# mbzuai-oryx/Video-LLaVA

Measured on NVIDIA H100. Metric: videos/sec (100-frame CLIP encode + 7B 32-tok decode), higher is better.
Workload: dtype bf16

## Files before the change

### video-llava_b200/csrc/attention_tc.cu

```cuda
#include "common.cuh"
#include "kernels.h"

#include <stdlib.h>

namespace vcl {

namespace {

constexpr int VA_WG = 2;
constexpr int VA_THREADS = VA_WG * 128;
constexpr int VA_TILE = 64 * 128;
constexpr int VA_KEY_TILES = 5;
constexpr int VA_OFF_K = 0;
constexpr int VA_OFF_VT = VA_OFF_K + VA_KEY_TILES * VA_TILE;
constexpr int VA_OFF_Q = VA_OFF_VT + VA_KEY_TILES * VA_TILE;
constexpr int VA_OFF_P = VA_OFF_Q + VA_WG * VA_TILE;
constexpr int VA_OFF_BAR = VA_OFF_P + VA_WG * VA_KEY_TILES * VA_TILE;
constexpr int VA_SMEM = VA_OFF_BAR + 64 + 1024;
static_assert(VA_SMEM <= 227 * 1024, "shared memory");

__device__ __forceinline__ uint32_t va_sw128(int row, int chunk) {
  return (uint32_t)row * 128u + (uint32_t)((chunk ^ (row & 7)) << 4);
}

__device__ __forceinline__ void named_bar_sync_wg(int id) { asm volatile("bar.sync %0, 128;" ::"r"(id) : "memory"); }

__global__ void __launch_bounds__(VA_THREADS, 1)
attn_vit_tc_kernel(const __grid_constant__ CUtensorMap tmap, const bf16* __restrict__ qkv, bf16* __restrict__ out,
                   int S, int H, int C) {
  extern __shared__ uint8_t smem_raw[];
  const uint32_t raw_addr = smem_u32(smem_raw);
  const uint32_t pad = ((raw_addr + 1023u) & ~1023u) - raw_addr;
  uint8_t* smem = smem_raw + pad;
  const uint32_t sbase = raw_addr + pad;
  const uint32_t kbar = sbase + VA_OFF_BAR;
  auto qbar = [&](int w) { return sbase + VA_OFF_BAR + 8u * (1 + w); };

  const int frame = blockIdx.x / H, h = blockIdx.x - frame * H;
  const int row0 = frame * S;
  const int wg = threadIdx.x >> 7, t = threadIdx.x & 127, lane = threadIdx.x & 31, wq = t >> 5;
  const int n_qt = (S + 63) / 64;
  const int n_kt = (S + 63) / 64;

  if (threadIdx.x == 0) {
    tma_prefetch_desc(&tmap);
    mbar_init(kbar, 1);
    for (int w = 0; w < VA_WG; ++w) mbar_init(qbar(w), 1);
    mbar_fence_init();
  }
  __syncthreads();
  if (threadIdx.x == 0) {
    mbar_arrive_expect_tx(kbar, n_kt * VA_TILE);
    for (int i = 0; i < n_kt; ++i) tma_load_2d(sbase + VA_OFF_K + i * VA_TILE, &tmap, kbar, C + h * 64, row0 + 64 * i);
    for (int w = 0; w < VA_WG && w < n_qt; ++w) {
      mbar_arrive_expect_tx(qbar(w), VA_TILE);
      tma_load_2d(sbase + VA_OFF_Q + w * VA_TILE, &tmap, qbar(w), h * 64, row0 + 64 * w);
    }
  }
  const bf16* vg = qkv + (long long)row0 * 3 * C + 2 * C + h * 64;
  for (int idx = threadIdx.x; idx < VA_KEY_TILES * 64 * 8; idx += VA_THREADS) {
    const int key = idx % (VA_KEY_TILES * 64), c = idx / (VA_KEY_TILES * 64);
    uint4 v = make_uint4(0u, 0u, 0u, 0u);
    if (key < S) v = *reinterpret_cast<const uint4*>(vg + (long long)key * 3 * C + c * 8);
    const uint32_t w4[4] = {v.x, v.y, v.z, v.w};
    uint8_t* tile = smem + VA_OFF_VT + (key >> 6) * VA_TILE;
    const int kc = (key & 63) >> 3, ke = key & 7;
#pragma unroll
    for (int e = 0; e < 8; ++e) {
      const uint16_t hv = (uint16_t)(e & 1 ? w4[e >> 1] >> 16 : w4[e >> 1] & 0xffffu);
      *reinterpret_cast<uint16_t*>(tile + va_sw128(c * 8 + e, kc) + ke * 2) = hv;
    }
  }
  asm volatile("fence.proxy.async.shared::cta;" ::: "memory");
  __syncthreads();
  mbar_wait(kbar, 0);

  const int r0 = 16 * wq + (lane >> 2), c2 = 2 * (lane & 3);
  const bool tail = S > 256;
  uint8_t* P = smem + VA_OFF_P + wg * VA_KEY_TILES * VA_TILE;
  const uint32_t p_addr = sbase + VA_OFF_P + wg * VA_KEY_TILES * VA_TILE;
  const uint32_t q_addr = sbase + VA_OFF_Q + wg * VA_TILE;
  uint32_t qphase = 0;
  float s[128], s2[16], o[32];
  for (int qt = wg; qt < n_qt; qt += VA_WG) {
    mbar_wait(qbar(wg), qphase);
    qphase ^= 1u;
#pragma unroll
    for (int i = 0; i < 128; ++i) s[i] = 0.f;
#pragma unroll
    for (int i = 0; i < 16; ++i) s2[i] = 0.f;
    wgmma_fence();
#pragma unroll
    for (int k = 0; k < 4; ++k) {
      const uint64_t ad = wgmma_desc_k_sw128(q_addr) + 2u * k;
      wgmma_bf16<256>(s, ad, wgmma_desc_k_sw128(sbase + VA_OFF_K) + 2u * k, k > 0 ? 1u : 0u);
      if (tail) wgmma_bf16<32>(s2, ad, wgmma_desc_k_sw128(sbase + VA_OFF_K + 256 * 128) + 2u * k, k > 0 ? 1u : 0u);
    }
    wgmma_commit();
    wgmma_wait<0>();
    wgmma_fence_regs(s);
    wgmma_fence_regs(s2);
    named_bar_sync_wg(1 + wg);
    if (t == 0 && qt + VA_WG < n_qt) {
      mbar_arrive_expect_tx(qbar(wg), VA_TILE);
      tma_load_2d(q_addr, &tmap, qbar(wg), h * 64, row0 + 64 * (qt + VA_WG));
    }
    auto sc = [&](float x, int key) { return key < S ? bf16r(bf16r(x) * 0.125f) : -INFINITY; };
    float m[2] = {-INFINITY, -INFINITY};
    uint32_t sp[64], sp2[8];
    auto pack_sc = [&](const float* a, int i, int key0) {
      const int hh = i & 1, col = key0 + 8 * (i >> 1) + c2;
      const float x0 = sc(a[2 * i], col), x1 = sc(a[2 * i + 1], col + 1);
      m[hh] = fmaxf(m[hh], fmaxf(x0, x1));
      return pack_bf16x2(x0, x1);
    };
    if (tail) {
#pragma unroll
      for (int i = 0; i < 8; ++i) sp2[i] = pack_sc(s2, i, 256);
    }
#pragma unroll
    for (int i = 0; i < 64; ++i) sp[i] = pack_sc(s, i, 0);
    float l[2] = {0.f, 0.f};
#pragma unroll
    for (int r = 0; r < 2; ++r) {
      m[r] = fmaxf(m[r], __shfl_xor_sync(0xffffffffu, m[r], 1));
      m[r] = fmaxf(m[r], __shfl_xor_sync(0xffffffffu, m[r], 2));
    }
    auto put_p = [&](uint32_t x2, int i, int key0) {
      const int hh = i & 1, row = r0 + 8 * hh, col = key0 + 8 * (i >> 1) + c2;
      const float p0 = exp2f((bf16lo(x2) - m[hh]) * 1.4426950408889634f);
      const float p1 = exp2f((bf16hi(x2) - m[hh]) * 1.4426950408889634f);
      l[hh] += p0 + p1;
      *reinterpret_cast<uint32_t*>(P + (col >> 6) * VA_TILE + va_sw128(row, (col & 63) >> 3) + (col & 7) * 2) =
          pack_bf16x2(p0, p1);
    };
#pragma unroll
    for (int i = 0; i < 64; ++i) put_p(sp[i], i, 0);
    if (tail) {
#pragma unroll
      for (int i = 0; i < 8; ++i) put_p(sp2[i], i, 256);
    }
    asm volatile("fence.proxy.async.shared::cta;" ::: "memory");
    named_bar_sync_wg(1 + wg);
#pragma unroll
    for (int i = 0; i < 32; ++i) o[i] = 0.f;
    wgmma_fence();
#pragma unroll
    for (int kk = 0; kk < 16; ++kk)
      wgmma_bf16<64>(o, wgmma_desc_k_sw128(p_addr + (kk >> 2) * VA_TILE) + 2u * (kk & 3),
                     wgmma_desc_k_sw128(sbase + VA_OFF_VT + (kk >> 2) * VA_TILE) + 2u * (kk & 3), kk > 0 ? 1u : 0u);
    if (tail)
      wgmma_bf16<64>(o, wgmma_desc_k_sw128(p_addr + 4 * VA_TILE), wgmma_desc_k_sw128(sbase + VA_OFF_VT + 4 * VA_TILE), 1u);
    wgmma_commit();
    wgmma_wait<0>();
    wgmma_fence_regs(o);
#pragma unroll
    for (int r = 0; r < 2; ++r) {
      l[r] += __shfl_xor_sync(0xffffffffu, l[r], 1);
      l[r] += __shfl_xor_sync(0xffffffffu, l[r], 2);
    }
#pragma unroll
    for (int hh = 0; hh < 2; ++hh) {
      const int q = qt * 64 + r0 + 8 * hh;
      if (q < S) {
        const float inv = 1.0f / l[hh];
        bf16* dst = out + (long long)(row0 + q) * C + h * 64 + c2;
#pragma unroll
        for (int j = 0; j < 8; ++j)
          *reinterpret_cast<uint32_t*>(dst + 8 * j) = pack_bf16x2(o[4 * j + 2 * hh] * inv, o[4 * j + 2 * hh + 1] * inv);
      }
    }
  }
}

}

int init_attention_tc_kernels() {
  VCL_CUDA_OK(cudaFuncSetAttribute(attn_vit_tc_kernel, cudaFuncAttributeMaxDynamicSharedMemorySize, VA_SMEM));
  return 0;
}

bool attention_vit_tc_supported(int S) {
  const bool off = getenv("VCL_VIT_ATTN_FLASH") != nullptr;
  return !off && S >= 129 && S <= 257;
}

int launch_attention_vit_tc(const bf16* qkv, bf16* out, int n_frames, int S, int H, int C, cudaStream_t stream) {
  VCL_REQUIRE(C == H * 64, "attention_vit_tc: head_dim must be 64");
  VCL_REQUIRE(S >= 129 && S <= 257, "attention_vit_tc: S=%d outside 129..257", S);
  VCL_REQUIRE(((uintptr_t)qkv % 16) == 0 && ((uintptr_t)out % 16) == 0, "attention_vit_tc: pointers must be 16-byte aligned");
  CUtensorMap tm;
  if (make_tmap_2d(&tm, qkv, (long long)n_frames * S, 3LL * C, 3LL * C, 64) != 0) return -2;
  attn_vit_tc_kernel<<<n_frames * H, VA_THREADS, VA_SMEM, stream>>>(tm, qkv, out, S, H, C);
  VCL_CUDA_OK(cudaGetLastError());
  count_launches(1);
  return 0;
}

}
```

### video-llava_b200/csrc/common.cuh

```cuda
#pragma once

#include <cuda.h>
#include <cuda_bf16.h>
#include <cuda_fp16.h>
#include <cuda_runtime.h>
#include <stdint.h>

namespace vcl {

typedef __nv_bfloat16 bf16;

void set_last_error(const char* fmt, ...);

#define VCL_CUDA_OK(expr)                                                                      \
  do {                                                                                         \
    cudaError_t _e = (expr);                                                                   \
    if (_e != cudaSuccess) {                                                                   \
      ::vcl::set_last_error("%s:%d: %s -> %s", __FILE__, __LINE__, #expr, cudaGetErrorString(_e)); \
      return -2;                                                                               \
    }                                                                                          \
  } while (0)

#define VCL_REQUIRE(cond, ...)                 \
  do {                                         \
    if (!(cond)) {                             \
      ::vcl::set_last_error(__VA_ARGS__);      \
      return -1;                               \
    }                                          \
  } while (0)

__device__ __forceinline__ float bf16r(float x) { return __bfloat162float(__float2bfloat16_rn(x)); }

__device__ __forceinline__ uint32_t pack_bf16x2(float lo, float hi) {
  __nv_bfloat162 v = __floats2bfloat162_rn(lo, hi);
  return *reinterpret_cast<uint32_t*>(&v);
}
__device__ __forceinline__ float act_sigmoid_div(float num, float x) {
  const float d = 1.0f + __expf(-x);
  const float s = d > 0x1p126f ? 0.25f : 1.0f;
  return __fdividef(num * s, d * s);
}
__device__ __forceinline__ float bf16lo(uint32_t v) { return __uint_as_float(v << 16); }
__device__ __forceinline__ float bf16hi(uint32_t v) { return __uint_as_float(v & 0xffff0000u); }

__device__ __forceinline__ uint32_t bf16x2_mul(uint32_t a, uint32_t b) {
  __nv_bfloat162 r = __hmul2(*reinterpret_cast<__nv_bfloat162*>(&a), *reinterpret_cast<__nv_bfloat162*>(&b));
  return *reinterpret_cast<uint32_t*>(&r);
}
__device__ __forceinline__ uint32_t bf16x2_add(uint32_t a, uint32_t b) {
  __nv_bfloat162 r = __hadd2(*reinterpret_cast<__nv_bfloat162*>(&a), *reinterpret_cast<__nv_bfloat162*>(&b));
  return *reinterpret_cast<uint32_t*>(&r);
}

__device__ __forceinline__ float warp_sum(float v) {
#pragma unroll
  for (int o = 16; o > 0; o >>= 1) v += __shfl_xor_sync(0xffffffffu, v, o);
  return v;
}
__device__ __forceinline__ float warp_max(float v) {
#pragma unroll
  for (int o = 16; o > 0; o >>= 1) v = fmaxf(v, __shfl_xor_sync(0xffffffffu, v, o));
  return v;
}

__device__ __forceinline__ uint4 ld_nc_v4(const void* p) {
  uint4 r;
  asm volatile("ld.global.nc.L1::no_allocate.v4.u32 {%0,%1,%2,%3}, [%4];"
               : "=r"(r.x), "=r"(r.y), "=r"(r.z), "=r"(r.w)
               : "l"(p));
  return r;
}

__device__ __forceinline__ uint32_t smem_u32(const void* p) {
  return static_cast<uint32_t>(__cvta_generic_to_shared(p));
}

__device__ __forceinline__ void mbar_init(uint32_t bar, uint32_t count) {
  asm volatile("mbarrier.init.shared::cta.b64 [%0], %1;" ::"r"(bar), "r"(count) : "memory");
}
__device__ __forceinline__ void mbar_fence_init() {
  asm volatile("fence.mbarrier_init.release.cluster;" ::: "memory");
  asm volatile("fence.proxy.async.shared::cta;" ::: "memory");
}
__device__ __forceinline__ void mbar_arrive_expect_tx(uint32_t bar, uint32_t bytes) {
  asm volatile("mbarrier.arrive.expect_tx.shared::cta.b64 _, [%0], %1;" ::"r"(bar), "r"(bytes)
               : "memory");
}
__device__ __forceinline__ void mbar_arrive(uint32_t bar) {
  asm volatile("mbarrier.arrive.shared::cta.b64 _, [%0];" ::"r"(bar) : "memory");
}
__device__ __forceinline__ void mbar_wait(uint32_t bar, uint32_t parity) {
  asm volatile(
      "{\n\t"
      ".reg .pred p;\n\t"
      "VCL_WAIT_%=:\n\t"
      "mbarrier.try_wait.parity.shared::cta.b64 p, [%0], %1;\n\t"
      "@p bra VCL_DONE_%=;\n\t"
      "bra VCL_WAIT_%=;\n\t"
      "VCL_DONE_%=:\n\t"
      "}\n" ::"r"(bar),
      "r"(parity)
      : "memory");
}

__device__ __forceinline__ void tma_prefetch_desc(const void* tmap) {
  asm volatile("prefetch.tensormap [%0];" ::"l"(tmap) : "memory");
}
__device__ __forceinline__ void tma_load_2d(uint32_t dst_smem, const void* tmap, uint32_t bar,
                                            int32_t c0, int32_t c1) {
  asm volatile(
      "cp.async.bulk.tensor.2d.shared::cluster.global.mbarrier::complete_tx::bytes"
      " [%0], [%1, {%3, %4}], [%2];" ::"r"(dst_smem),
      "l"(tmap), "r"(bar), "r"(c0), "r"(c1)
      : "memory");
}

__device__ __forceinline__ void tma_prefetch_2d(const void* tmap, int32_t c0, int32_t c1) {
  asm volatile("cp.async.bulk.prefetch.tensor.2d.L2.global.tile [%0, {%1, %2}];" ::"l"(tmap), "r"(c0), "r"(c1)
               : "memory");
}

__device__ __forceinline__ void tma_load_2d_mc(uint32_t dst_smem, const void* tmap, uint32_t bar,
                                               int32_t c0, int32_t c1, uint16_t cta_mask) {
  asm volatile(
      "cp.async.bulk.tensor.2d.shared::cluster.global.mbarrier::complete_tx::bytes.multicast::cluster"
      " [%0], [%1, {%3, %4}], [%2], %5;" ::"r"(dst_smem),
      "l"(tmap), "r"(bar), "r"(c0), "r"(c1), "h"(cta_mask)
      : "memory");
}

__device__ __forceinline__ uint32_t cluster_ctarank() {
  uint32_t r;
  asm volatile("mov.u32 %0, %%cluster_ctarank;" : "=r"(r));
  return r;
}
__device__ __forceinline__ void cluster_sync_all() {
  asm volatile("barrier.cluster.arrive.release.aligned;" ::: "memory");
  asm volatile("barrier.cluster.wait.acquire.aligned;" ::: "memory");
}

__device__ __forceinline__ uint32_t mapa_cluster(uint32_t smem_addr, uint32_t cta_rank) {
  uint32_t r;
  asm volatile("mapa.shared::cluster.u32 %0, %1, %2;" : "=r"(r) : "r"(smem_addr), "r"(cta_rank));
  return r;
}
__device__ __forceinline__ void mbar_arrive_cluster(uint32_t bar_cluster_addr) {
  asm volatile("mbarrier.arrive.release.cluster.shared::cluster.b64 _, [%0];" ::"r"(bar_cluster_addr) : "memory");
}

__device__ __forceinline__ void wgmma_fence() { asm volatile("wgmma.fence.sync.aligned;" ::: "memory"); }
__device__ __forceinline__ void wgmma_commit() { asm volatile("wgmma.commit_group.sync.aligned;" ::: "memory"); }
template <int N>
__device__ __forceinline__ void wgmma_wait() {
  asm volatile("wgmma.wait_group.sync.aligned %0;" ::"n"(N) : "memory");
}
template <int R>
__device__ __forceinline__ void wgmma_fence_regs(float (&d)[R]) {
#pragma unroll
  for (int i = 0; i < R; ++i) asm volatile("" : "+f"(d[i])::"memory");
}
template <int R>
__device__ __forceinline__ void setmaxnreg_inc() { asm volatile("setmaxnreg.inc.sync.aligned.u32 %0;" ::"n"(R)); }
template <int R>
__device__ __forceinline__ void setmaxnreg_dec() { asm volatile("setmaxnreg.dec.sync.aligned.u32 %0;" ::"n"(R)); }

__device__ __forceinline__ uint64_t wgmma_desc_k_sw128(uint32_t smem_addr) {
  uint64_t d = 0;
  d |= (uint64_t)((smem_addr & 0x3ffffu) >> 4);
  d |= (uint64_t)1 << 16;
  d |= (uint64_t)(1024u >> 4) << 32;
  d |= (uint64_t)1 << 62;
  return d;
}

template <int N>
__device__ __forceinline__ void wgmma_bf16(float (&d)[N / 2], uint64_t adesc, uint64_t bdesc, uint32_t accumulate);
template <>
__device__ __forceinline__ void wgmma_bf16<256>(float (&d)[128], uint64_t adesc, uint64_t bdesc, uint32_t accumulate) {
  asm volatile(
      "{\n\t.reg .pred p;\n\tsetp.ne.b32 p, %130, 0;\n\t"
      "wgmma.mma_async.sync.aligned.m64n256k16.f32.bf16.bf16 {%0, %1, %2, %3, %4, %5, %6, %7, %8, %9, %10, %11, %12, %13, %14, %15, %16, %17, %18, %19, %20, %21, %22, %23, %24, %25, %26, %27, %28, %29, %30, %31, %32, %33, %34, %35, %36, %37, %38, %39, %40, %41, %42, %43, %44, %45, %46, %47, %48, %49, %50, %51, %52, %53, %54, %55, %56, %57, %58, %59, %60, %61, %62, %63, %64, %65, %66, %67, %68, %69, %70, %71, %72, %73, %74, %75, %76, %77, %78, %79, %80, %81, %82, %83, %84, %85, %86, %87, %88, %89, %90, %91, %92, %93, %94, %95, %96, %97, %98, %99, %100, %101, %102, %103, %104, %105, %106, %107, %108, %109, %110, %111, %112, %113, %114, %115, %116, %117, %118, %119, %120, %121, %122, %123, %124, %125, %126, %127}, %128, %129, p, 1, 1, 0, 0;\n\t}"
      : "+f"(d[0]), "+f"(d[1]), "+f"(d[2]), "+f"(d[3]), "+f"(d[4]), "+f"(d[5]), "+f"(d[6]), "+f"(d[7]), "+f"(d[8]), "+f"(d[9]), "+f"(d[10]), "+f"(d[11]), "+f"(d[12]), "+f"(d[13]), "+f"(d[14]), "+f"(d[15]), "+f"(d[16]), "+f"(d[17]), "+f"(d[18]), "+f"(d[19]), "+f"(d[20]), "+f"(d[21]), "+f"(d[22]), "+f"(d[23]), "+f"(d[24]), "+f"(d[25]), "+f"(d[26]), "+f"(d[27]), "+f"(d[28]), "+f"(d[29]), "+f"(d[30]), "+f"(d[31]), "+f"(d[32]), "+f"(d[33]), "+f"(d[34]), "+f"(d[35]), "+f"(d[36]), "+f"(d[37]), "+f"(d[38]), "+f"(d[39]), "+f"(d[40]), "+f"(d[41]), "+f"(d[42]), "+f"(d[43]), "+f"(d[44]), "+f"(d[45]), "+f"(d[46]), "+f"(d[47]), "+f"(d[48]), "+f"(d[49]), "+f"(d[50]), "+f"(d[51]), "+f"(d[52]), "+f"(d[53]), "+f"(d[54]), "+f"(d[55]), "+f"(d[56]), "+f"(d[57]), "+f"(d[58]), "+f"(d[59]), "+f"(d[60]), "+f"(d[61]), "+f"(d[62]), "+f"(d[63]), "+f"(d[64]), "+f"(d[65]), "+f"(d[66]), "+f"(d[67]), "+f"(d[68]), "+f"(d[69]), "+f"(d[70]), "+f"(d[71]), "+f"(d[72]), "+f"(d[73]), "+f"(d[74]), "+f"(d[75]), "+f"(d[76]), "+f"(d[77]), "+f"(d[78]), "+f"(d[79]), "+f"(d[80]), "+f"(d[81]), "+f"(d[82]), "+f"(d[83]), "+f"(d[84]), "+f"(d[85]), "+f"(d[86]), "+f"(d[87]), "+f"(d[88]), "+f"(d[89]), "+f"(d[90]), "+f"(d[91]), "+f"(d[92]), "+f"(d[93]), "+f"(d[94]), "+f"(d[95]), "+f"(d[96]), "+f"(d[97]), "+f"(d[98]), "+f"(d[99]), "+f"(d[100]), "+f"(d[101]), "+f"(d[102]), "+f"(d[103]), "+f"(d[104]), "+f"(d[105]), "+f"(d[106]), "+f"(d[107]), "+f"(d[108]), "+f"(d[109]), "+f"(d[110]), "+f"(d[111]), "+f"(d[112]), "+f"(d[113]), "+f"(d[114]), "+f"(d[115]), "+f"(d[116]), "+f"(d[117]), "+f"(d[118]), "+f"(d[119]), "+f"(d[120]), "+f"(d[121]), "+f"(d[122]), "+f"(d[123]), "+f"(d[124]), "+f"(d[125]), "+f"(d[126]), "+f"(d[127])
      : "l"(adesc), "l"(bdesc), "r"(accumulate));
}
template <>
__device__ __forceinline__ void wgmma_bf16<128>(float (&d)[64], uint64_t adesc, uint64_t bdesc, uint32_t accumulate) {
  asm volatile(
      "{\n\t.reg .pred p;\n\tsetp.ne.b32 p, %66, 0;\n\t"
      "wgmma.mma_async.sync.aligned.m64n128k16.f32.bf16.bf16 {%0, %1, %2, %3, %4, %5, %6, %7, %8, %9, %10, %11, %12, %13, %14, %15, %16, %17, %18, %19, %20, %21, %22, %23, %24, %25, %26, %27, %28, %29, %30, %31, %32, %33, %34, %35, %36, %37, %38, %39, %40, %41, %42, %43, %44, %45, %46, %47, %48, %49, %50, %51, %52, %53, %54, %55, %56, %57, %58, %59, %60, %61, %62, %63}, %64, %65, p, 1, 1, 0, 0;\n\t}"
      : "+f"(d[0]), "+f"(d[1]), "+f"(d[2]), "+f"(d[3]), "+f"(d[4]), "+f"(d[5]), "+f"(d[6]), "+f"(d[7]), "+f"(d[8]), "+f"(d[9]), "+f"(d[10]), "+f"(d[11]), "+f"(d[12]), "+f"(d[13]), "+f"(d[14]), "+f"(d[15]), "+f"(d[16]), "+f"(d[17]), "+f"(d[18]), "+f"(d[19]), "+f"(d[20]), "+f"(d[21]), "+f"(d[22]), "+f"(d[23]), "+f"(d[24]), "+f"(d[25]), "+f"(d[26]), "+f"(d[27]), "+f"(d[28]), "+f"(d[29]), "+f"(d[30]), "+f"(d[31]), "+f"(d[32]), "+f"(d[33]), "+f"(d[34]), "+f"(d[35]), "+f"(d[36]), "+f"(d[37]), "+f"(d[38]), "+f"(d[39]), "+f"(d[40]), "+f"(d[41]), "+f"(d[42]), "+f"(d[43]), "+f"(d[44]), "+f"(d[45]), "+f"(d[46]), "+f"(d[47]), "+f"(d[48]), "+f"(d[49]), "+f"(d[50]), "+f"(d[51]), "+f"(d[52]), "+f"(d[53]), "+f"(d[54]), "+f"(d[55]), "+f"(d[56]), "+f"(d[57]), "+f"(d[58]), "+f"(d[59]), "+f"(d[60]), "+f"(d[61]), "+f"(d[62]), "+f"(d[63])
      : "l"(adesc), "l"(bdesc), "r"(accumulate));
}
template <>
__device__ __forceinline__ void wgmma_bf16<64>(float (&d)[32], uint64_t adesc, uint64_t bdesc, uint32_t accumulate) {
  asm volatile(
      "{\n\t.reg .pred p;\n\tsetp.ne.b32 p, %34, 0;\n\t"
      "wgmma.mma_async.sync.aligned.m64n64k16.f32.bf16.bf16 {%0, %1, %2, %3, %4, %5, %6, %7, %8, %9, %10, %11, %12, %13, %14, %15, %16, %17, %18, %19, %20, %21, %22, %23, %24, %25, %26, %27, %28, %29, %30, %31}, %32, %33, p, 1, 1, 0, 0;\n\t}"
      : "+f"(d[0]), "+f"(d[1]), "+f"(d[2]), "+f"(d[3]), "+f"(d[4]), "+f"(d[5]), "+f"(d[6]), "+f"(d[7]), "+f"(d[8]), "+f"(d[9]), "+f"(d[10]), "+f"(d[11]), "+f"(d[12]), "+f"(d[13]), "+f"(d[14]), "+f"(d[15]), "+f"(d[16]), "+f"(d[17]), "+f"(d[18]), "+f"(d[19]), "+f"(d[20]), "+f"(d[21]), "+f"(d[22]), "+f"(d[23]), "+f"(d[24]), "+f"(d[25]), "+f"(d[26]), "+f"(d[27]), "+f"(d[28]), "+f"(d[29]), "+f"(d[30]), "+f"(d[31])
      : "l"(adesc), "l"(bdesc), "r"(accumulate));
}
template <>
__device__ __forceinline__ void wgmma_bf16<32>(float (&d)[16], uint64_t adesc, uint64_t bdesc, uint32_t accumulate) {
  asm volatile(
      "{\n\t.reg .pred p;\n\tsetp.ne.b32 p, %18, 0;\n\t"
      "wgmma.mma_async.sync.aligned.m64n32k16.f32.bf16.bf16 {%0, %1, %2, %3, %4, %5, %6, %7, %8, %9, %10, %11, %12, %13, %14, %15}, %16, %17, p, 1, 1, 0, 0;\n\t}"
      : "+f"(d[0]), "+f"(d[1]), "+f"(d[2]), "+f"(d[3]), "+f"(d[4]), "+f"(d[5]), "+f"(d[6]), "+f"(d[7]), "+f"(d[8]), "+f"(d[9]), "+f"(d[10]), "+f"(d[11]), "+f"(d[12]), "+f"(d[13]), "+f"(d[14]), "+f"(d[15])
      : "l"(adesc), "l"(bdesc), "r"(accumulate));
}

}
```

### video-llava_b200/csrc/gemm_tc.cu

```cuda
#include "common.cuh"
#include "kernels.h"

#include <cudaTypedefs.h>

namespace vcl {

template <int BLOCK_N>
struct GemmCfg {
  static constexpr int BLOCK_M = 128;
  static constexpr int BLOCK_K = 64;
  static constexpr int A_BYTES = BLOCK_M * BLOCK_K * 2;
  static constexpr int B_BYTES = BLOCK_N * BLOCK_K * 2;
  static constexpr int STAGE_BYTES = A_BYTES + B_BYTES;
  static constexpr int OUT_PITCH = BLOCK_N * 2 + 16;
  static constexpr int OUT_BYTES = BLOCK_M * OUT_PITCH;
  static constexpr int BAR_BYTES = 256;
  static constexpr int STAGES = (BLOCK_N == 256) ? 3 : (BLOCK_N == 128 ? 5 : 8);
  static constexpr int SMEM_BYTES = STAGES * STAGE_BYTES + BAR_BYTES + OUT_BYTES + 1024;
  static_assert((2 * STAGES + 4) * 8 <= BAR_BYTES, "barrier area");
  static_assert(SMEM_BYTES <= 227 * 1024, "shared memory");
};

__device__ __forceinline__ float act_gelu_erf(float x) {
  x = bf16r(x);
// ... 225 lines not shown
    }
  } else {
    setmaxnreg_inc<224>();
    const int cw = wg - 1;
    const int t = threadIdx.x & 127, lane = threadIdx.x & 31, wq = t >> 5;
    uint8_t* stg = stage_out + cw * 64 * Cfg::OUT_PITCH;
    auto release = [&](int s) {
      if (t == 0) {
        if (CL == 1) {
          mbar_arrive(empty_bar(s));
        } else {
#pragma unroll
          for (int r = 0; r < CL; ++r) mbar_arrive_cluster(mapa_cluster(empty_bar(s), (uint32_t)r));
        }
      }
    };
    float acc[BLOCK_N / 2];
    int stage = 0;
    uint32_t phase = 0, out_phase = 0;
    for (int tile = cluster_id; tile < num_tiles; tile += n_clusters) {
      const int m_blk = (tile / num_n) * CL + cta_rank, n_blk = tile % num_n;
      int prev = -1;
      for (int kb = 0; kb < num_k; ++kb) {
        mbar_wait(full_bar(stage), phase);
        const uint32_t a_addr = smem_base + stage * Cfg::STAGE_BYTES;
        const uint64_t a_desc = wgmma_desc_k_sw128(a_addr + cw * 64 * 128);
        const uint64_t b_desc = wgmma_desc_k_sw128(a_addr + Cfg::A_BYTES);
        wgmma_fence();
#pragma unroll
        for (int k = 0; k < Cfg::BLOCK_K / 16; ++k) {
          wgmma_bf16<BLOCK_N>(acc, a_desc + 2u * k, b_desc + 2u * k, (kb | k) != 0 ? 1u : 0u);
        }
        wgmma_commit();
        wgmma_wait<1>();
        if (prev >= 0) release(prev);
        prev = stage;
        if (++stage == STAGES) { stage = 0; phase ^= 1u; }
      }
      wgmma_wait<0>();
      release(prev);
      wgmma_fence_regs(acc);
      if (tile != cluster_id) {
        mbar_wait(drained_bar(cw), out_phase);
        out_phase ^= 1u;
      }
      gemm_epilogue_stage<BLOCK_N, ACT>(acc, stg, lane, wq, m_blk * Cfg::BLOCK_M + cw * 64, n_blk, bias, M, N, rope);
      mbar_arrive(staged_bar(cw));
    }
  }

  __syncthreads();
  if (CL > 1) cluster_sync_all();
}

static PFN_cuTensorMapEncodeTiled_v12000 g_encode = nullptr;
static int resolve_encode() {
  if (g_encode) return 0;
  void* fn = nullptr;
  cudaDriverEntryPointQueryResult qres;
  cudaError_t e = cudaGetDriverEntryPoint("cuTensorMapEncodeTiled", &fn, cudaEnableDefault, &qres);
  if (e != cudaSuccess || fn == nullptr || qres != cudaDriverEntryPointSuccess) {
    set_last_error("cuTensorMapEncodeTiled is not available from the driver (%s)",
                   cudaGetErrorString(e));
    return -2;
  }
  g_encode = reinterpret_cast<PFN_cuTensorMapEncodeTiled_v12000>(fn);
  return 0;
}

int make_tmap_2d(CUtensorMap* out, const void* ptr, long long rows, long long cols, long long ld,
                 int box_rows) {
  if (resolve_encode() != 0) return -2;
  cuuint64_t gdim[2] = {(cuuint64_t)cols, (cuuint64_t)rows};
  cuuint64_t gstride[1] = {(cuuint64_t)ld * 2};
  cuuint32_t box[2] = {64u, (cuuint32_t)box_rows};
  cuuint32_t estr[2] = {1u, 1u};
  CUresult r = g_encode(out, CU_TENSOR_MAP_DATA_TYPE_BFLOAT16, 2, const_cast<void*>(ptr), gdim,
                        gstride, box, estr, CU_TENSOR_MAP_INTERLEAVE_NONE,
                        CU_TENSOR_MAP_SWIZZLE_128B, CU_TENSOR_MAP_L2_PROMOTION_L2_256B,
                        CU_TENSOR_MAP_FLOAT_OOB_FILL_NONE);
  if (r != CUDA_SUCCESS) {
    set_last_error("cuTensorMapEncodeTiled failed (%d) ptr=%p rows=%lld cols=%lld ld=%lld box=%d",
                   (int)r, ptr, rows, cols, ld, box_rows);
    return -2;
  }
  return 0;
}

static int g_num_sms = 0;
int device_num_sms() {
  if (g_num_sms == 0) {
    int dev = 0;
    cudaGetDevice(&dev);
    cudaDeviceGetAttribute(&g_num_sms, cudaDevAttrMultiProcessorCount, dev);
    if (g_num_sms <= 0) g_num_sms = 132;
  }
  return g_num_sms;
}

template <int BLOCK_N, int ACT, int CL>
static int launch_one(const GemmArgs& g, cudaStream_t stream) {
  using Cfg = GemmCfg<BLOCK_N>;
  auto kern = gemm_bf16_tn_kernel<BLOCK_N, ACT, CL>;
  CUtensorMap ta, tb;
  if (make_tmap_2d(&ta, g.A, g.M, g.K, g.lda, Cfg::BLOCK_M) != 0) return -2;
  if (make_tmap_2d(&tb, g.W, g.N, g.K, g.ldw, BLOCK_N / CL) != 0) return -2;
  const int num_m = (g.M + 127) / 128;
  const int num_tiles = ((num_m + CL - 1) / CL) * ((g.N + BLOCK_N - 1) / BLOCK_N);
  cudaLaunchConfig_t cfg = {};
  cfg.blockDim = dim3(384);
  cfg.dynamicSmemBytes = Cfg::SMEM_BYTES;
  cfg.stream = stream;
  cudaLaunchAttribute attr[1];
  attr[0].id = cudaLaunchAttributeClusterDimension;
  attr[0].val.clusterDim.x = CL;
  attr[0].val.clusterDim.y = 1;
  attr[0].val.clusterDim.z = 1;
  cfg.attrs = attr;
  cfg.numAttrs = CL > 1 ? 1 : 0;
  static int resident = 0;
  if (resident == 0) {
    if (CL > 1) {
      cfg.gridDim = dim3(CL);
      VCL_CUDA_OK(cudaOccupancyMaxActiveClusters(&resident, kern, &cfg));
    }
    if (resident <= 0) resident = device_num_sms() / CL;
  }
  int clusters = resident;
  if (clusters > num_tiles) clusters = num_tiles;
  if (g.max_ctas > 0 && clusters * CL > g.max_ctas) clusters = g.max_ctas / CL > 0 ? g.max_ctas / CL : 1;
  cfg.gridDim = dim3(clusters * CL);
  VCL_CUDA_OK(cudaLaunchKernelEx(&cfg, kern, ta, tb, g.C, (long long)g.ldc, g.bias, g.residual,
                                 (long long)g.ldr, g.M, g.N, g.K, g.rope));
  count_launches(1);
  return 0;
}

template <int BLOCK_N, int ACT>
static int launch_cl(const GemmArgs& g, int cl, cudaStream_t stream) {
  if (BLOCK_N >= 128) {
    if (cl == 4) return launch_one<BLOCK_N, ACT, (BLOCK_N >= 128 ? 4 : 1)>(g, stream);
    if (cl == 2) return launch_one<BLOCK_N, ACT, (BLOCK_N >= 128 ? 2 : 1)>(g, stream);
  }
  return launch_one<BLOCK_N, ACT, 1>(g, stream);
}

template <int BLOCK_N>
static int launch_act(const GemmArgs& g, int cl, cudaStream_t stream) {
  switch (g.act) {
    case ACT_NONE: return launch_cl<BLOCK_N, ACT_NONE>(g, cl, stream);
    case ACT_QGELU: return launch_cl<BLOCK_N, ACT_QGELU>(g, cl, stream);
    case ACT_GELU: return launch_cl<BLOCK_N, ACT_GELU>(g, cl, stream);
    case ACT_SWIGLU: return launch_cl<BLOCK_N, ACT_SWIGLU>(g, cl, stream);
    case ACT_ROPE:
      if constexpr (BLOCK_N >= 128) return launch_cl<BLOCK_N, ACT_ROPE>(g, cl, stream);
      break;
  }
  set_last_error("gemm: unknown activation %d", g.act);
  return -1;
}

template <int BLOCK_N, int ACT>
static int init_one() {
  VCL_CUDA_OK(cudaFuncSetAttribute(gemm_bf16_tn_kernel<BLOCK_N, ACT, 1>,
                                   cudaFuncAttributeMaxDynamicSharedMemorySize,
                                   GemmCfg<BLOCK_N>::SMEM_BYTES));
// ... 77 lines not shown
```

### video-llava_b200/csrc/kernels.h

```cpp
#pragma once

#include <cuda.h>
#include <cuda_bf16.h>
#include <cuda_runtime.h>
#include <stdint.h>

namespace vcl {

typedef __nv_bfloat16 bf16;

constexpr int PACK_SEQ_MAX = 64;
constexpr int PACK_HEAD = 6 * PACK_SEQ_MAX;
inline size_t pack_elems(long long rows) { return PACK_HEAD + 2 * (size_t)rows; }
template <class T> __host__ __device__ inline T* pack_off(T* p) { return p; }
template <class T> __host__ __device__ inline T* pack_len(T* p) { return p + PACK_SEQ_MAX; }
template <class T> __host__ __device__ inline T* pack_slot(T* p) { return p + 2 * PACK_SEQ_MAX; }
template <class T> __host__ __device__ inline T* pack_last(T* p) { return p + 3 * PACK_SEQ_MAX; }
template <class T> __host__ __device__ inline T* pack_start(T* p) { return p + 4 * PACK_SEQ_MAX; }
template <class T> __host__ __device__ inline T* pack_end(T* p) { return p + 5 * PACK_SEQ_MAX; }
template <class T> __host__ __device__ inline T* pack_row(T* p, long long r) { return p + PACK_HEAD + 2 * r; }

struct KvPages {
  const int* table = nullptr;
  int row = 0;
  long long blk = 0;
};
__device__ __forceinline__ long long kv_paged_off(const KvPages& p, int slot, int head, int col) {
  return (long long)__ldg(p.table + slot * p.row + (col >> 7)) * p.blk + ((long long)head * 128 + (col & 127)) * 128;
}

enum Act { ACT_NONE = 0, ACT_QGELU = 1, ACT_GELU = 2, ACT_SWIGLU = 3, ACT_ROPE = 4 };
struct RopeEpilogue {
  const bf16* cos_t = nullptr; const bf16* sin_t = nullptr;
  bf16* kcache = nullptr; bf16* vcache = nullptr;
  int S = 0, start_pos = 0, H = 0, s_max = 0;
  const int* n_pad = nullptr;
  const int* pack = nullptr;
  KvPages pages;
};


void set_last_error(const char* fmt, ...);
void count_launches(long long n);
long long launch_count();
int device_num_sms();

struct GemmArgs {
  const bf16* A = nullptr;  long long lda = 0;
  const bf16* W = nullptr;  long long ldw = 0;
  bf16* C = nullptr;        long long ldc = 0;
  const bf16* bias = nullptr;
  const bf16* residual = nullptr; long long ldr = 0;
  int M = 0, N = 0, K = 0;
  int act = ACT_NONE;
  int block_n = 0;
  int cluster = 0;
  int max_ctas = 0;
  RopeEpilogue rope;
};
int launch_gemm_bf16_tn(const GemmArgs& g, cudaStream_t stream);
int init_gemm_kernels();
int make_tmap_2d(CUtensorMap* out, const void* ptr, long long rows, long long cols, long long ld,
                 int box_rows);

int launch_layernorm(const bf16* x, long long ldx, bf16* y, long long ldy, const bf16* w,
                     const bf16* b, int rows, int D, float eps, cudaStream_t stream);
int launch_rmsnorm(const bf16* x, long long ldx, bf16* y, long long ldy, const bf16* w, int rows,
                   int D, float eps, cudaStream_t stream);
int launch_im2col(const void* pixels, int mode, bf16* out, int n_frames, int image, int patch,
                  int KP, cudaStream_t stream);
int launch_clip_embed_ln(const bf16* patch_out, const bf16* cls, const bf16* pos, const bf16* ln_w,
                         const bf16* ln_b, bf16* h, int n_frames, int P, int D, float eps,
                         cudaStream_t stream);
int launch_embed_splice(const long long* ids, const bf16* table, const bf16* vid, const int* vid_start,
                        bf16* h, int B, int S, int D, int n_vid, int vocab, cudaStream_t stream,
                        const int* pack = nullptr, int M = 0);
int launch_rope_table(bf16* cos_t, bf16* sin_t, int max_pos, int head_dim, float theta,
                      cudaStream_t stream);
int launch_rope_kv_prefill(bf16* qkv, bf16* kcache, bf16* vcache, const bf16* cos_t,
                           const bf16* sin_t, int B, int S, int H, int head_dim, int s_max, int pos0,
                           cudaStream_t stream, const int* pos_dev = nullptr, const int* n_pad = nullptr);
int launch_embed_tokens(const int* tok, long long tok_stride, const bf16* table, bf16* h, int B,
                        int D, int vocab, cudaStream_t stream);
int launch_argmax(const float* logits, int* out, long long out_stride, int B, int V,
                  cudaStream_t stream);
int launch_fill_int(int* dst, int value, int n, cudaStream_t stream);

int launch_st_pool(const void* feats, int in_dtype, long long frame_stride, long long patch_stride,
                   int T, int P, int C, int n_temporal, void* out, int out_dtype,
                   cudaStream_t stream);

size_t resize_frames_workspace(int n, int in_h, int in_w, int mode, int out_h, int out_w, int crop_top, int crop_left,
                               int crop_h, int crop_w);
int launch_resize_frames(const uint8_t* in, int n, int in_h, int in_w, int mode, int out_h, int out_w, int crop_top,
                         int crop_left, int crop_h, int crop_w, uint8_t* out, void* ws, size_t ws_bytes,
                         cudaStream_t stream);

int launch_cross_entropy(const bf16* logits, long long ld, int V, const long long* labels, long long row0, int rows,
                         int seg, float* nll, bf16* logits_out, cudaStream_t stream);
int launch_nll_mean(const float* nll, const long long* labels, long long rows, int seg, float* nll_out,
                    float* loss_out, cudaStream_t stream);
int launch_label_logprobs(const bf16* logits, long long ld, int V, const long long* labels, int rows, float* lp,
                          uint8_t* greedy, cudaStream_t stream);

#ifndef VCL_LOGPROBS_MAX
#define VCL_LOGPROBS_MAX 20
#endif
#ifndef VCL_SAMPLE_WIDE_MAX_V
#define VCL_SAMPLE_WIDE_MAX_V 57344
#endif
struct SampleArgs {
  const float* logits = nullptr; long long ld = 0; int V = 0, B = 0;
  const float* temperature = nullptr; const int* top_k = nullptr; const unsigned long long* seed = nullptr;
  int entry0 = 0; const int* rowmap = nullptr;
  int col = 0; const int* col_dev = nullptr; const int* n_pad = nullptr;
  int* out = nullptr; long long out_stride = 1;
  const int* top_n = nullptr;
  int* lp_id = nullptr; float* lp_val = nullptr;
  long long lp_entry = 0, lp_pos = 0; int lp_rows = 0;
  const float* top_p = nullptr; const float* rep = nullptr;
  unsigned int* tset = nullptr; int tset_words = 0;
  int* hist = nullptr; long long hist_ld = 0;
  const int* bans = nullptr;
};
#ifndef VCL_BAN_WORDS_MAX
#define VCL_BAN_WORDS_MAX 1024
#endif
constexpr int VCL_BAN_ROW = 4 + VCL_BAN_WORDS_MAX;
int launch_sample(const SampleArgs& a, cudaStream_t stream);
int launch_token_history(int* dst, const long long* ids, int n, cudaStream_t stream);
int launch_token_set(unsigned int* dst, int words, const long long* ids, int n, int V, cudaStream_t stream);

#ifndef VCL_BEAM_MAX
#define VCL_BEAM_MAX 8
#endif
struct BeamRec { float score; int beam; int token; };
struct BeamArgs {
  const float* logits = nullptr; long long ld = 0; int V = 0;
  int B = 0, k = 0, first = 0, step = 0;
  const int* ctl = nullptr;
  const float* score = nullptr; float* score_out = nullptr;
  int* map = nullptr; int* tok_out = nullptr; int2* fork = nullptr;
  BeamRec* rec = nullptr; int* pick = nullptr;
  unsigned int* cand_key = nullptr; int* cand_tok = nullptr;
};
int launch_beam_select(const BeamArgs& a, cudaStream_t stream);
// ... 89 lines not shown
```

Before: 5.042.

## Make ViT attention kernel persistent with warp-specialized TMA producer and register-sourced PV

Rewrites the ViT attention kernel as a persistent, warp-specialized kernel. A producer warp streams K, V and Q through double-buffered shared memory with a 3D per-frame tensor map and mbarriers. Consumer warpgroups keep P in registers and feed it to register-sourced wgmma, replacing the manual V transpose and the P shared-memory round trip. Tail handling becomes a template parameter and the max reduction moves to packed bf16. This aims to overlap loads with compute and cut shared-memory traffic and launch granularity, at the cost of more complex barrier and phase logic and register pressure.

```diff
diff --git a/video-llava_b200/csrc/attention_tc.cu b/video-llava_b200/csrc/attention_tc.cu
--- a/video-llava_b200/csrc/attention_tc.cu
+++ b/video-llava_b200/csrc/attention_tc.cu
@@ -8,83 +8,92 @@
 namespace {
 
 constexpr int VA_WG = 2;
-constexpr int VA_THREADS = VA_WG * 128;
+constexpr int VA_THREADS = VA_WG * 128 + 128;
 constexpr int VA_TILE = 64 * 128;
 constexpr int VA_KEY_TILES = 5;
+constexpr int VA_STAGES = 2;
+constexpr int VA_QSLOTS = 2;
 constexpr int VA_OFF_K = 0;
-constexpr int VA_OFF_VT = VA_OFF_K + VA_KEY_TILES * VA_TILE;
-constexpr int VA_OFF_Q = VA_OFF_VT + VA_KEY_TILES * VA_TILE;
-constexpr int VA_OFF_P = VA_OFF_Q + VA_WG * VA_TILE;
-constexpr int VA_OFF_BAR = VA_OFF_P + VA_WG * VA_KEY_TILES * VA_TILE;
-constexpr int VA_SMEM = VA_OFF_BAR + 64 + 1024;
+constexpr int VA_OFF_V = VA_OFF_K + VA_STAGES * VA_KEY_TILES * VA_TILE;
+constexpr int VA_OFF_Q = VA_OFF_V + VA_STAGES * VA_KEY_TILES * VA_TILE;
+constexpr int VA_OFF_BAR = VA_OFF_Q + VA_WG * VA_QSLOTS * VA_TILE;
+constexpr int VA_BAR_K = 0, VA_BAR_V = VA_STAGES, VA_BAR_KVE = 2 * VA_STAGES, VA_BAR_Q = 3 * VA_STAGES,
+              VA_BAR_QE = VA_BAR_Q + VA_WG * VA_QSLOTS, VA_NBAR = VA_BAR_QE + VA_WG * VA_QSLOTS;
+constexpr int VA_SMEM = VA_OFF_BAR + 8 * VA_NBAR + 1024;
 static_assert(VA_SMEM <= 227 * 1024, "shared memory");
 
-__device__ __forceinline__ uint32_t va_sw128(int row, int chunk) {
-  return (uint32_t)row * 128u + (uint32_t)((chunk ^ (row & 7)) << 4);
-}
-
-__device__ __forceinline__ void named_bar_sync_wg(int id) { asm volatile("bar.sync %0, 128;" ::"r"(id) : "memory"); }
-
+template <bool TAIL>
 __global__ void __launch_bounds__(VA_THREADS, 1)
-attn_vit_tc_kernel(const __grid_constant__ CUtensorMap tmap, const bf16* __restrict__ qkv, bf16* __restrict__ out,
-                   int S, int H, int C) {
+attn_vit_tc_kernel(const __grid_constant__ CUtensorMap tmap, bf16* __restrict__ out, int n_frames, int S, int H,
+                   int C) {
   extern __shared__ uint8_t smem_raw[];
   const uint32_t raw_addr = smem_u32(smem_raw);
-  const uint32_t pad = ((raw_addr + 1023u) & ~1023u) - raw_addr;
-  uint8_t* smem = smem_raw + pad;
-  const uint32_t sbase = raw_addr + pad;
-  const uint32_t kbar = sbase + VA_OFF_BAR;
-  auto qbar = [&](int w) { return sbase + VA_OFF_BAR + 8u * (1 + w); };
-
-  const int frame = blockIdx.x / H, h = blockIdx.x - frame * H;
-  const int row0 = frame * S;
-  const int wg = threadIdx.x >> 7, t = threadIdx.x & 127, lane = threadIdx.x & 31, wq = t >> 5;
+  const uint32_t sbase = (raw_addr + 1023u) & ~1023u;
+  auto bar = [&](int i) { return sbase + VA_OFF_BAR + 8u * i; };
+
+  const int n_items = n_frames * H;
   const int n_qt = (S + 63) / 64;
-  const int n_kt = (S + 63) / 64;
+  const int n_kt = TAIL ? 5 : 4;
 
   if (threadIdx.x == 0) {
     tma_prefetch_desc(&tmap);
-    mbar_init(kbar, 1);
-    for (int w = 0; w < VA_WG; ++w) mbar_init(qbar(w), 1);
+    for (int s = 0; s < VA_STAGES; ++s) {
+      mbar_init(bar(VA_BAR_K + s), 1);
+      mbar_init(bar(VA_BAR_V + s), 1);
+      mbar_init(bar(VA_BAR_KVE + s), VA_WG * 128);
+    }
+    for (int i = 0; i < VA_WG * VA_QSLOTS; ++i) {
+      mbar_init(bar(VA_BAR_Q + i), 1);
+      mbar_init(bar(VA_BAR_QE + i), 128);
+    }
     mbar_fence_init();
   }
   __syncthreads();
-  if (threadIdx.x == 0) {
-    mbar_arrive_expect_tx(kbar, n_kt * VA_TILE);
-    for (int i = 0; i < n_kt; ++i) tma_load_2d(sbase + VA_OFF_K + i * VA_TILE, &tmap, kbar, C + h * 64, row0 + 64 * i);
-    for (int w = 0; w < VA_WG && w < n_qt; ++w) {
-      mbar_arrive_expect_tx(qbar(w), VA_TILE);
-      tma_load_2d(sbase + VA_OFF_Q + w * VA_TILE, &tmap, qbar(w), h * 64, row0 + 64 * w);
-    }
+
+  if (threadIdx.x >= VA_WG * 128) {
+    setmaxnreg_dec<24>();
+    if (threadIdx.x != VA_WG * 128) return;
+    for (int j = 0;; ++j) {
+      const int item = blockIdx.x + j * gridDim.x;
+      if (item >= n_items) break;
+      const int frame = item / H, h = item - frame * H;
+      const int st = j & 1, use = j >> 1;
+      if (use > 0) mbar_wait(bar(VA_BAR_KVE + st), (use - 1) & 1);
+      const uint32_t kdst = sbase + VA_OFF_K + st * VA_KEY_TILES * VA_TILE;
+      const uint32_t vdst = sbase + VA_OFF_V + st * VA_KEY_TILES * VA_TILE;
+      mbar_arrive_expect_tx(bar(VA_BAR_K + st), n_kt * VA_TILE);
+      for (int i = 0; i < n_kt; ++i) tma_load_3d(kdst + i * VA_TILE, &tmap, bar(VA_BAR_K + st), C + h * 64, 64 * i, frame);
+      mbar_arrive_expect_tx(bar(VA_BAR_V + st), n_kt * VA_TILE);
+      for (int i = 0; i < n_kt; ++i)
+        tma_load_3d(vdst + i * VA_TILE, &tmap, bar(VA_BAR_V + st), 2 * C + h * 64, 64 * i, frame);
+      for (int qt = 0; qt < n_qt; ++qt) {
+        const int g = j * n_qt + qt, w = g & 1, t = g >> 1;
+        const int slot = w * VA_QSLOTS + (t & 1), quse = t >> 1;
+        if (quse > 0) mbar_wait(bar(VA_BAR_QE + slot), (quse - 1) & 1);
+        mbar_arrive_expect_tx(bar(VA_BAR_Q + slot), VA_TILE);
+        tma_load_3d(sbase + VA_OFF_Q + slot * VA_TILE, &tmap, bar(VA_BAR_Q + slot), h * 64, 64 * qt, frame);
+      }
+    }
+    return;
   }
-  const bf16* vg = qkv + (long long)row0 * 3 * C + 2 * C + h * 64;
-  for (int idx = threadIdx.x; idx < VA_KEY_TILES * 64 * 8; idx += VA_THREADS) {
-    const int key = idx % (VA_KEY_TILES * 64), c = idx / (VA_KEY_TILES * 64);
-    uint4 v = make_uint4(0u, 0u, 0u, 0u);
-    if (key < S) v = *reinterpret_cast<const uint4*>(vg + (long long)key * 3 * C + c * 8);
-    const uint32_t w4[4] = {v.x, v.y, v.z, v.w};
-    uint8_t* tile = smem + VA_OFF_VT + (key >> 6) * VA_TILE;
-    const int kc = (key & 63) >> 3, ke = key & 7;
-#pragma unroll
-    for (int e = 0; e < 8; ++e) {
-      const uint16_t hv = (uint16_t)(e & 1 ? w4[e >> 1] >> 16 : w4[e >> 1] & 0xffffu);
-      *reinterpret_cast<uint16_t*>(tile + va_sw128(c * 8 + e, kc) + ke * 2) = hv;
-    }
-  }
-  asm volatile("fence.proxy.async.shared::cta;" ::: "memory");
-  __syncthreads();
-  mbar_wait(kbar, 0);
-
+
+  setmaxnreg_inc<240>();
+  const int wg = threadIdx.x >> 7, t128 = threadIdx.x & 127, lane = threadIdx.x & 31, wq = t128 >> 5;
   const int r0 = 16 * wq + (lane >> 2), c2 = 2 * (lane & 3);
-  const bool tail = S > 256;
-  uint8_t* P = smem + VA_OFF_P + wg * VA_KEY_TILES * VA_TILE;
-  const uint32_t p_addr = sbase + VA_OFF_P + wg * VA_KEY_TILES * VA_TILE;
-  const uint32_t q_addr = sbase + VA_OFF_Q + wg * VA_TILE;
-  uint32_t qphase = 0;
   float s[128], s2[16], o[32];
-  for (int qt = wg; qt < n_qt; qt += VA_WG) {
-    mbar_wait(qbar(wg), qphase);
-    qphase ^= 1u;
+  for (int t = 0;; ++t) {
+    const int g = 2 * t + wg, j = g / n_qt, qt = g - j * n_qt;
+    const int item = blockIdx.x + j * gridDim.x;
+    if (item >= n_items) break;
+    const int frame = item / H, h = item - frame * H;
+    const int st = j & 1;
+    const uint32_t kvpar = (j >> 1) & 1;
+    const int slot = wg * VA_QSLOTS + (t & 1);
+    const uint32_t k_addr = sbase + VA_OFF_K + st * VA_KEY_TILES * VA_TILE;
+    const uint32_t v_addr = sbase + VA_OFF_V + st * VA_KEY_TILES * VA_TILE;
+    const uint32_t q_addr = sbase + VA_OFF_Q + slot * VA_TILE;
+    mbar_wait(bar(VA_BAR_K + st), kvpar);
+    mbar_wait(bar(VA_BAR_Q + slot), (t >> 1) & 1);
 #pragma unroll
     for (int i = 0; i < 128; ++i) s[i] = 0.f;
 #pragma unroll
@@ -93,72 +102,79 @@
 #pragma unroll
     for (int k = 0; k < 4; ++k) {
       const uint64_t ad = wgmma_desc_k_sw128(q_addr) + 2u * k;
-      wgmma_bf16<256>(s, ad, wgmma_desc_k_sw128(sbase + VA_OFF_K) + 2u * k, k > 0 ? 1u : 0u);
-      if (tail) wgmma_bf16<32>(s2, ad, wgmma_desc_k_sw128(sbase + VA_OFF_K + 256 * 128) + 2u * k, k > 0 ? 1u : 0u);
+      wgmma_bf16<256>(s, ad, wgmma_desc_k_sw128(k_addr) + 2u * k, k > 0 ? 1u : 0u);
+      if constexpr (TAIL) wgmma_bf16<32>(s2, ad, wgmma_desc_k_sw128(k_addr + 256 * 128) + 2u * k, k > 0 ? 1u : 0u);
     }
     wgmma_commit();
     wgmma_wait<0>();
     wgmma_fence_regs(s);
     wgmma_fence_regs(s2);
-    named_bar_sync_wg(1 + wg);
-    if (t == 0 && qt + VA_WG < n_qt) {
-      mbar_arrive_expect_tx(qbar(wg), VA_TILE);
-      tma_load_2d(q_addr, &tmap, qbar(wg), h * 64, row0 + 64 * (qt + VA_WG));
-    }
-    auto sc = [&](float x, int key) { return key < S ? bf16r(bf16r(x) * 0.125f) : -INFINITY; };
-    float m[2] = {-INFINITY, -INFINITY};
-    uint32_t sp[64], sp2[8];
-    auto pack_sc = [&](const float* a, int i, int key0) {
+    mbar_arrive(bar(VA_BAR_QE + slot));
+    uint32_t mx[2] = {0xff80ff80u, 0xff80ff80u};
+    uint32_t p[64], p2[8];
+    auto pack_sc = [&](const float* a, int i, int key0, bool masked) {
       const int hh = i & 1, col = key0 + 8 * (i >> 1) + c2;
-      const float x0 = sc(a[2 * i], col), x1 = sc(a[2 * i + 1], col + 1);
-      m[hh] = fmaxf(m[hh], fmaxf(x0, x1));
-      return pack_bf16x2(x0, x1);
+      uint32_t x2 = bf16x2_mul(pack_bf16x2(a[2 * i], a[2 * i + 1]), 0x3e003e00u);
+      if (masked) {
+        if (col >= S) x2 = (x2 & 0xffff0000u) | 0xff80u;
+        if (col + 1 >= S) x2 = (x2 & 0x0000ffffu) | 0xff800000u;
+      }
+      mx[hh] = bf16x2_max(mx[hh], x2);
+      return x2;
     };
-    if (tail) {
-#pragma unroll
-      for (int i = 0; i < 8; ++i) sp2[i] = pack_sc(s2, i, 256);
-    }
-#pragma unroll
-    for (int i = 0; i < 64; ++i) sp[i] = pack_sc(s, i, 0);
-    float l[2] = {0.f, 0.f};
+    if constexpr (TAIL) {
+#pragma unroll
+      for (int i = 0; i < 8; ++i) p2[i] = pack_sc(s2, i, 256, true);
+    }
+#pragma unroll
+    for (int i = 0; i < 64; ++i) p[i] = pack_sc(s, i, 0, !TAIL);
+    float m[2], l[2] = {0.f, 0.f};
 #pragma unroll
     for (int r = 0; r < 2; ++r) {
+      m[r] = fmaxf(bf16lo(mx[r]), bf16hi(mx[r]));
       m[r] = fmaxf(m[r], __shfl_xor_sync(0xffffffffu, m[r], 1));
       m[r] = fmaxf(m[r], __shfl_xor_sync(0xffffffffu, m[r], 2));
     }
-    auto put_p = [&](uint32_t x2, int i, int key0) {
-      const int hh = i & 1, row = r0 + 8 * hh, col = key0 + 8 * (i >> 1) + c2;
+    auto weight = [&](uint32_t x2, int i) {
+      const int hh = i & 1;
       const float p0 = exp2f((bf16lo(x2) - m[hh]) * 1.4426950408889634f);
       const float p1 = exp2f((bf16hi(x2) - m[hh]) * 1.4426950408889634f);
       l[hh] += p0 + p1;
-      *reinterpret_cast<uint32_t*>(P + (col >> 6) * VA_TILE + va_sw128(row, (col & 63) >> 3) + (col & 7) * 2) =
-          pack_bf16x2(p0, p1);
+      return pack_bf16x2(p0, p1);
     };
 #pragma unroll
-    for (int i = 0; i < 64; ++i) put_p(sp[i], i, 0);
-    if (tail) {
-#pragma unroll
-      for (int i = 0; i < 8; ++i) put_p(sp2[i], i, 256);
-    }
-    asm volatile("fence.proxy.async.shared::cta;" ::: "memory");
-    named_bar_sync_wg(1 + wg);
+    for (int i = 0; i < 64; ++i) p[i] = weight(p[i], i);
+    if constexpr (TAIL) {
+#pragma unroll
+      for (int i = 0; i < 8; ++i) p2[i] = weight(p2[i], i);
+    }
+    mbar_wait(bar(VA_BAR_V + st), kvpar);
 #pragma unroll
     for (int i = 0; i < 32; ++i) o[i] = 0.f;
     wgmma_fence();
 #pragma unroll
-    for (int kk = 0; kk < 16; ++kk)
-      wgmma_bf16<64>(o, wgmma_desc_k_sw128(p_addr + (kk >> 2) * VA_TILE) + 2u * (kk & 3),
-                     wgmma_desc_k_sw128(sbase + VA_OFF_VT + (kk >> 2) * VA_TILE) + 2u * (kk & 3), kk > 0 ? 1u : 0u);
-    if (tail)
-      wgmma_bf16<64>(o, wgmma_desc_k_sw128(p_addr + 4 * VA_TILE), wgmma_desc_k_sw128(sbase + VA_OFF_VT + 4 * VA_TILE), 1u);
+    for (int kk = 0; kk < 16; ++kk) {
+      const uint32_t a[4] = {p[4 * kk], p[4 * kk + 1], p[4 * kk + 2], p[4 * kk + 3]};
+      wgmma_bf16_rs_n64_tb(o, a, wgmma_desc_k_sw128(v_addr + (kk >> 2) * VA_TILE + (kk & 3) * 2048), kk > 0 ? 1u : 0u);
+    }
+    if constexpr (TAIL) {
+      const uint32_t a[4] = {p2[0], p2[1], p2[2], p2[3]};
+      wgmma_bf16_rs_n64_tb(o, a, wgmma_desc_k_sw128(v_addr + 4 * VA_TILE), 1u);
+    }
     wgmma_commit();
     wgmma_wait<0>();
     wgmma_fence_regs(o);
 #pragma unroll
+    for (int i = 0; i < 64; ++i) asm volatile("" ::"r"(p[i]) : "memory");
+#pragma unroll
+    for (int i = 0; i < 8; ++i) asm volatile("" ::"r"(p2[i]) : "memory");
+    if ((g + 2) / n_qt != j) mbar_arrive(bar(VA_BAR_KVE + st));
+#pragma unroll
     for (int r = 0; r < 2; ++r) {
       l[r] += __shfl_xor_sync(0xffffffffu, l[r], 1);
       l[r] += __shfl_xor_sync(0xffffffffu, l[r], 2);
     }
+    const int row0 = frame * S;
 #pragma unroll
     for (int hh = 0; hh < 2; ++hh) {
       const int q = qt * 64 + r0 + 8 * hh;
@@ -166,8 +182,8 @@
         const float inv = 1.0f / l[hh];
         bf16* dst = out + (long long)(row0 + q) * C + h * 64 + c2;
 #pragma unroll
-        for (int j = 0; j < 8; ++j)
-          *reinterpret_cast<uint32_t*>(dst + 8 * j) = pack_bf16x2(o[4 * j + 2 * hh] * inv, o[4 * j + 2 * hh + 1] * inv);
+        for (int j8 = 0; j8 < 8; ++j8)
+          *reinterpret_cast<uint32_t*>(dst + 8 * j8) = pack_bf16x2(o[4 * j8 + 2 * hh] * inv, o[4 * j8 + 2 * hh + 1] * inv);
       }
     }
   }
@@ -176,7 +192,8 @@
 }
 
 int init_attention_tc_kernels() {
-  VCL_CUDA_OK(cudaFuncSetAttribute(attn_vit_tc_kernel, cudaFuncAttributeMaxDynamicSharedMemorySize, VA_SMEM));
+  VCL_CUDA_OK(cudaFuncSetAttribute(attn_vit_tc_kernel<false>, cudaFuncAttributeMaxDynamicSharedMemorySize, VA_SMEM));
+  VCL_CUDA_OK(cudaFuncSetAttribute(attn_vit_tc_kernel<true>, cudaFuncAttributeMaxDynamicSharedMemorySize, VA_SMEM));
   return 0;
 }
 
@@ -190,8 +207,12 @@
   VCL_REQUIRE(S >= 129 && S <= 257, "attention_vit_tc: S=%d outside 129..257", S);
   VCL_REQUIRE(((uintptr_t)qkv % 16) == 0 && ((uintptr_t)out % 16) == 0, "attention_vit_tc: pointers must be 16-byte aligned");
   CUtensorMap tm;
-  if (make_tmap_2d(&tm, qkv, (long long)n_frames * S, 3LL * C, 3LL * C, 64) != 0) return -2;
-  attn_vit_tc_kernel<<<n_frames * H, VA_THREADS, VA_SMEM, stream>>>(tm, qkv, out, S, H, C);
+  if (make_tmap_frames(&tm, qkv, n_frames, S, 3LL * C, 3LL * C, 64) != 0) return -2;
+  const int grid = n_frames * H < device_num_sms() ? n_frames * H : device_num_sms();
+  if (S > 256)
+    attn_vit_tc_kernel<true><<<grid, VA_THREADS, VA_SMEM, stream>>>(tm, out, n_frames, S, H, C);
+  else
+    attn_vit_tc_kernel<false><<<grid, VA_THREADS, VA_SMEM, stream>>>(tm, out, n_frames, S, H, C);
   VCL_CUDA_OK(cudaGetLastError());
   count_launches(1);
   return 0;
diff --git a/video-llava_b200/csrc/common.cuh b/video-llava_b200/csrc/common.cuh
--- a/video-llava_b200/csrc/common.cuh
+++ b/video-llava_b200/csrc/common.cuh
@@ -49,6 +49,11 @@
 }
 __device__ __forceinline__ uint32_t bf16x2_add(uint32_t a, uint32_t b) {
   __nv_bfloat162 r = __hadd2(*reinterpret_cast<__nv_bfloat162*>(&a), *reinterpret_cast<__nv_bfloat162*>(&b));
+  return *reinterpret_cast<uint32_t*>(&r);
+}
+
+__device__ __forceinline__ uint32_t bf16x2_max(uint32_t a, uint32_t b) {
+  __nv_bfloat162 r = __hmax2(*reinterpret_cast<__nv_bfloat162*>(&a), *reinterpret_cast<__nv_bfloat162*>(&b));
   return *reinterpret_cast<uint32_t*>(&r);
 }
 
@@ -115,6 +120,15 @@
       : "memory");
 }
 
+__device__ __forceinline__ void tma_load_3d(uint32_t dst_smem, const void* tmap, uint32_t bar,
+                                            int32_t c0, int32_t c1, int32_t c2) {
+  asm volatile(
+      "cp.async.bulk.tensor.3d.shared::cluster.global.mbarrier::complete_tx::bytes"
+      " [%0], [%1, {%3, %4, %5}], [%2];" ::"r"(dst_smem),
+      "l"(tmap), "r"(bar), "r"(c0), "r"(c1), "r"(c2)
+      : "memory");
+}
+
 __device__ __forceinline__ void tma_prefetch_2d(const void* tmap, int32_t c0, int32_t c1) {
   asm volatile("cp.async.bulk.prefetch.tensor.2d.L2.global.tile [%0, {%1, %2}];" ::"l"(tmap), "r"(c0), "r"(c1)
                : "memory");
@@ -208,4 +222,13 @@
       : "l"(adesc), "l"(bdesc), "r"(accumulate));
 }
 
-}
+__device__ __forceinline__ void wgmma_bf16_rs_n64_tb(float (&d)[32], const uint32_t (&a)[4], uint64_t bdesc,
+                                                     uint32_t accumulate) {
+  asm volatile(
+      "{\n\t.reg .pred p;\n\tsetp.ne.b32 p, %37, 0;\n\t"
+      "wgmma.mma_async.sync.aligned.m64n64k16.f32.bf16.bf16 {%0, %1, %2, %3, %4, %5, %6, %7, %8, %9, %10, %11, %12, %13, %14, %15, %16, %17, %18, %19, %20, %21, %22, %23, %24, %25, %26, %27, %28, %29, %30, %31}, {%32, %33, %34, %35}, %36, p, 1, 1, 1;\n\t}"
+      : "+f"(d[0]), "+f"(d[1]), "+f"(d[2]), "+f"(d[3]), "+f"(d[4]), "+f"(d[5]), "+f"(d[6]), "+f"(d[7]), "+f"(d[8]), "+f"(d[9]), "+f"(d[10]), "+f"(d[11]), "+f"(d[12]), "+f"(d[13]), "+f"(d[14]), "+f"(d[15]), "+f"(d[16]), "+f"(d[17]), "+f"(d[18]), "+f"(d[19]), "+f"(d[20]), "+f"(d[21]), "+f"(d[22]), "+f"(d[23]), "+f"(d[24]), "+f"(d[25]), "+f"(d[26]), "+f"(d[27]), "+f"(d[28]), "+f"(d[29]), "+f"(d[30]), "+f"(d[31])
+      : "r"(a[0]), "r"(a[1]), "r"(a[2]), "r"(a[3]), "l"(bdesc), "r"(accumulate));
+}
+
+}
diff --git a/video-llava_b200/csrc/gemm_tc.cu b/video-llava_b200/csrc/gemm_tc.cu
--- a/video-llava_b200/csrc/gemm_tc.cu
+++ b/video-llava_b200/csrc/gemm_tc.cu
@@ -331,6 +331,25 @@
   if (r != CUDA_SUCCESS) {
     set_last_error("cuTensorMapEncodeTiled failed (%d) ptr=%p rows=%lld cols=%lld ld=%lld box=%d",
                    (int)r, ptr, rows, cols, ld, box_rows);
+    return -2;
+  }
+  return 0;
+}
+
+int make_tmap_frames(CUtensorMap* out, const void* ptr, long long frames, long long S, long long cols, long long ld,
+                     int box_rows) {
+  if (resolve_encode() != 0) return -2;
+  cuuint64_t gdim[3] = {(cuuint64_t)cols, (cuuint64_t)S, (cuuint64_t)frames};
+  cuuint64_t gstride[2] = {(cuuint64_t)ld * 2, (cuuint64_t)(ld * S) * 2};
+  cuuint32_t box[3] = {64u, (cuuint32_t)box_rows, 1u};
+  cuuint32_t estr[3] = {1u, 1u, 1u};
+  CUresult r = g_encode(out, CU_TENSOR_MAP_DATA_TYPE_BFLOAT16, 3, const_cast<void*>(ptr), gdim,
+                        gstride, box, estr, CU_TENSOR_MAP_INTERLEAVE_NONE,
+                        CU_TENSOR_MAP_SWIZZLE_128B, CU_TENSOR_MAP_L2_PROMOTION_L2_256B,
+                        CU_TENSOR_MAP_FLOAT_OOB_FILL_NONE);
+  if (r != CUDA_SUCCESS) {
+    set_last_error("cuTensorMapEncodeTiled failed (%d) ptr=%p frames=%lld S=%lld cols=%lld ld=%lld box=%d",
+                   (int)r, ptr, frames, S, cols, ld, box_rows);
     return -2;
   }
   return 0;
diff --git a/video-llava_b200/csrc/kernels.h b/video-llava_b200/csrc/kernels.h
--- a/video-llava_b200/csrc/kernels.h
+++ b/video-llava_b200/csrc/kernels.h
@@ -62,6 +62,8 @@
 int init_gemm_kernels();
 int make_tmap_2d(CUtensorMap* out, const void* ptr, long long rows, long long cols, long long ld,
                  int box_rows);
+int make_tmap_frames(CUtensorMap* out, const void* ptr, long long frames, long long S, long long cols, long long ld,
+                     int box_rows);
 
 int launch_layernorm(const bf16* x, long long ldx, bf16* y, long long ldy, const bf16* w,
                      const bf16* b, int rows, int D, float eps, cudaStream_t stream);
```

Result: faster. 5.129 (median of 6 runs) (+1.7%).
